# YooSungHyun/RNNTransducer

Hardware: AMD Instinct MI355X
Metric: utterances/sec (higher is better)
Workload: dtype f32

## Files before the change

### rnntransducer_amd/csrc/common.hpp

```cpp
#pragma once
#include <hip/hip_runtime.h>
#include <stdarg.h>
#include <stdint.h>
#include <stdio.h>

#include <atomic>

#include "rnnt_hip.h"

namespace rnnt {

void set_error(const char* fmt, ...);

#define RNNT_CHECK_ARG(cond, ...)      \
  do {                                 \
    if (!(cond)) {                     \
      ::rnnt::set_error(__VA_ARGS__);  \
      return RNNT_ERR_INVALID;         \
    }                                  \
  } while (0)

#define RNNT_CHECK_HIP(expr)                                                          \
  do {                                                                                \
    hipError_t e_ = (expr);                                                           \
// ... 2 lines not shown
      return RNNT_ERR_LAUNCH;                                                         \
    }                                                                                 \
  } while (0)

#define RNNT_CHECK_LAUNCH() RNNT_CHECK_HIP(hipGetLastError())

struct ProfScope {
  ProfScope(int kind, double work, hipStream_t s);
  ~ProfScope();
  int kind_;
  double work_;
  hipStream_t stream_;
  void* start_;
};

extern std::atomic<bool> g_launch_log_on;
void launch_log_note(const void* kernel, hipStream_t s);

static inline int64_t ceil_div(int64_t a, int64_t b) { return (a + b - 1) / b; }

int launch_colsum(const float* X, long M, long N, long ld, float* out, void* ws, size_t ws_bytes, hipStream_t s, int accumulate = 0);

size_t hp_plane_bytes(int64_t rows, int64_t K);
int hp_colmax(const float* x, int64_t rows, int64_t C, int64_t ld, uint32_t* amax, hipStream_t s);
int hp_split(const float* x, int64_t rows, int64_t K, int64_t ld, uint32_t* amax, void* planes, hipStream_t s, const int* rowidx = nullptr);
int hp_split_t(const float* x, int64_t R, int64_t K, int64_t ld, int64_t Ksrc, int64_t shift, const uint32_t* amax, void* planes,
               hipStream_t s, const int* kidx = nullptr);
int hp_split_both(const float* x, int64_t M, int64_t C, int64_t ld, const uint32_t* rowmax, const uint32_t* colmax, void* planes_rm,
                  void* planes_t, hipStream_t s, const int* rowidx = nullptr);
size_t hp_gemm_workspace_bytes(int64_t M, int64_t N, int64_t K);
int hp_gemm(const void* A, const uint32_t* a_amax, const void* B, const uint32_t* b_amax, int64_t M, int64_t N, int64_t K, float* C,
            int64_t c_div, int64_t c_so, int64_t c_si, const float* bias, unsigned flags, void* workspace, size_t workspace_bytes,
            hipStream_t s, const int* a_rowidx = nullptr, int64_t a_plane_rows = 0, const int* c_rowidx = nullptr);
struct HpProblem {
  const void* A; const uint32_t* a_amax; const void* B; const uint32_t* b_amax;
  int64_t M, N, K;
  float* C; int64_t ldc;
  unsigned flags;
};
constexpr int HP_GROUP_MAX = 4;
size_t hp_gemm_grouped_workspace_bytes(const int64_t* MN, int n);
int hp_gemm_grouped(const HpProblem* pr, int n, unsigned xcd_skip, unsigned* counter, void* workspace, size_t workspace_bytes,
                    hipStream_t s, unsigned* status = nullptr);
constexpr size_t HPQ_HEADER_BYTES = 256;
static inline size_t align_up(size_t a, size_t b) { return (a + b - 1) / b * b; }

__device__ __forceinline__ float gelu_tanh(float x) {
  const float k0 = 0.7978845608028654f, k1 = 0.044715f;
  float u = k0 * (x + k1 * x * x * x);
  return 0.5f * x * (1.0f + tanhf(u));
}
__device__ __forceinline__ float dgelu_tanh(float x) {
  const float k0 = 0.7978845608028654f, k1 = 0.044715f;
  float x2 = x * x;
  float u = k0 * (x + k1 * x * x2);
  float th = tanhf(u);
  float du = k0 * (1.0f + 3.0f * k1 * x2);
  return 0.5f * (1.0f + th) + 0.5f * x * (1.0f - th * th) * du;
}

__device__ __forceinline__ float sigmoidf_(float x) { return 1.0f / (1.0f + expf(-x)); }
__device__ __forceinline__ float tanh_e(float x) { return 1.0f - 2.0f / (expf(2.0f * x) + 1.0f); }
__device__ __forceinline__ float sigmoid_hw(float x) { return __builtin_amdgcn_rcpf(1.0f + __expf(-x)); }
__device__ __forceinline__ float tanh_hw(float x) { return 1.0f - 2.0f * __builtin_amdgcn_rcpf(__expf(2.0f * x) + 1.0f); }

typedef float f32x4 __attribute__((ext_vector_type(4)));
// ... 35 lines not shown
```

### rnntransducer_amd/csrc/gemm_hp.hip

```cpp
#include "common.hpp"

#include <stdlib.h>

namespace rnnt {
namespace {

typedef _Float16 f16x8 __attribute__((ext_vector_type(8)));
typedef __attribute__((address_space(3))) void lds_void;

constexpr int HP_BM = 256, HP_BN = 256, HP_BK = 32;
constexpr int HP_STAGE = (HP_BM + HP_BN) * 128;
constexpr int HP_RSRC = 0x00027000;

__device__ __forceinline__ float hp_scale_from_amax(unsigned amax_bits) {
  int eb = (int)((amax_bits >> 23) & 255u);
  if (eb == 0) return 1.0f;
  eb = eb < 15 ? 15 : eb;
  return __uint_as_float((unsigned)(268 - eb) << 23);
}
__device__ __forceinline__ float hp_inv_scale_from_amax(unsigned amax_bits) {
  int eb = (int)((amax_bits >> 23) & 255u);
  if (eb == 0) return 1.0f;
  eb = eb < 15 ? 15 : eb;
  return __uint_as_float((unsigned)(eb - 14) << 23);
// ... 391 lines not shown
      continue;
    }
#pragma unroll
    for (int ii = 0; ii < 4; ++ii) {
#pragma unroll
      for (int reg = 0; reg < 4; ++reg) {
        const int m = mrow + 16 * (4 * h + ii) + reg;
        const bool mok = m < p.M;
        const int mc = mok ? m : 0;
        float* crow = cbase + c_row(c_rowidx ? c_rowidx[mc] : mc);
        float old[4] = {0.f, 0.f, 0.f, 0.f};
        if (mode == 2) {
#pragma unroll
          for (int j = 0; j < 4; ++j)
            if (mok && nok[j]) old[j] = crow[ncol + 16 * j];
        }
#pragma unroll
        for (int j = 0; j < 4; ++j)
          if (mok && nok[j]) crow[ncol + 16 * j] = acc[4 * h + ii][j][reg] * sa[4 * ii + reg] * sb[j] + bias_v[j] + old[j];
      }
    }
  }
}

__device__ __forceinline__ int hp_grouped_tile(int idx, int tiles_m, int tiles_n, int group_m) {
  const int band = group_m * tiles_n;
  const int g = idx / band, r = idx - g * band;
  const int m_first = g * group_m;
  const int gm = min(tiles_m - m_first, group_m);
  const int n = r / gm, m = m_first + (r - n * gm);
  return n * tiles_m + m;
}

template <bool F16>
__global__ void __launch_bounds__(512, 1) gemm_hp_kernel(const HpGemmK p) {
  extern __shared__ __attribute__((aligned(16))) char lds[];
  int bid = hp_xcd_remap(blockIdx.x, p.tiles_m * p.tiles_n);
  if (p.group_m > 0) bid = hp_grouped_tile(bid, p.tiles_m, p.tiles_n, p.group_m);
  hp_tile256<F16, false>(p, bid, blockIdx.y, lds);
}

constexpr int HPQ_MAX = 4;
struct HpGemmQ {
  HpGemmK prob[HPQ_MAX];
  int unit_end[HPQ_MAX];
  int nprob;
  unsigned xcd_skip;
  unsigned* counter;
};

template <bool F16>
__global__ void __launch_bounds__(512, 1) gemm_hpq_kernel(const HpGemmQ q) {
  extern __shared__ __attribute__((aligned(16))) char lds[];
  unsigned xcc;
  asm volatile("s_getreg_b32 %0, hwreg(HW_REG_XCC_ID)" : "=s"(xcc));
  xcc &= 7u;
  if ((q.xcd_skip >> xcc) & 1u) return;
  const unsigned allow = ~q.xcd_skip & 0xffu;
  const int nq = __builtin_popcount(allow);
  const int mine = __builtin_popcount(allow & ((1u << xcc) - 1u));
  int* next = reinterpret_cast<int*>(lds + 2 * HP_STAGE);
  const int total = q.unit_end[q.nprob - 1];
  for (int hop = 0; hop < nq; ++hop) {
    const int qi = (mine + hop) % nq;
    const int lo = (int)((long)total * qi / nq), hi = (int)((long)total * (qi + 1) / nq);
    while (true) {
      if (threadIdx.x == 0) {
        const int got = lo + (int)atomicAdd(q.counter + qi, 1u);
        *next = got;
        if (got < hi) atomicAdd(q.counter + 8, 1u);
      }
      __syncthreads();
      const int u = __builtin_amdgcn_readfirstlane(*next);
      __syncthreads();
      if (u >= hi) break;
      int pi = 0;
      while (u >= q.unit_end[pi]) ++pi;
      const HpGemmK& p = q.prob[pi];
      const int local = u - (pi ? q.unit_end[pi - 1] : 0);
      const int tn = local % p.tiles_n, z = (local / p.tiles_n) % p.splits, tm = local / (p.tiles_n * p.splits);
      hp_tile256<F16, true>(p, tn * p.tiles_m + tm, z, lds);
    }
  }
}

__global__ void hpq_check_kernel(unsigned* counter, unsigned total, unsigned* status) {
  if (counter[8] != total) {
    counter[9] = 1u;
    if (status) __hip_atomic_store(status, 2u, __ATOMIC_RELAXED, __HIP_MEMORY_SCOPE_AGENT);
  }
}

__global__ void __launch_bounds__(256) hp_splitk_reduce_kernel(const HpGemmK p) {
  const long total = (long)p.M * p.N;
  for (long i = (long)blockIdx.x * 256 + threadIdx.x; i < total; i += (long)gridDim.x * 256) {
    const int m = (int)(i / p.N), n = (int)(i % p.N);
    float s = 0.f;
    for (int z = 0; z < p.splits; ++z) s += p.slab[(long)z * total + i];
    if (p.bias) s += p.bias[n];
    const int mo = p.c_rowidx ? p.c_rowidx[m] : m;
    const long off = (long)(mo / p.c_div) * p.c_so + (long)(mo % p.c_div) * p.c_si + n;
    if (p.flags & RNNT_GEMM_ACCUM) s += p.C[off];
    p.C[off] = s;
  }
}

}

size_t hp_plane_bytes(int64_t rows, int64_t K) { return (size_t)rows * (size_t)ceil_div(K, 32) * 128; }

int hp_colmax(const float* x, int64_t rows, int64_t C, int64_t ld, uint32_t* amax, hipStream_t s) {
  RNNT_CHECK_HIP(hipMemsetAsync(amax, 0, (size_t)C * 4, s));
  if (rows == 0 || C == 0) return RNNT_OK;
  long chunks = ceil_div(2048, ceil_div(C, 256));
  if (chunks > ceil_div(rows, 64)) chunks = ceil_div(rows, 64);
  if (chunks < 1) chunks = 1;
  const long rpc = ceil_div(rows, chunks);
  ProfScope prof(RNNT_K_HP_SPLIT, 4.0 * (double)rows * (double)C, s);
  hipLaunchKernelGGL(hp_colmax_kernel, dim3((unsigned)ceil_div(C, 256), (unsigned)ceil_div(rows, rpc)), dim3(256), 0, s, x, (long)rows, (int)C,
                     (long)ld, rpc, amax);
  RNNT_CHECK_LAUNCH();
  return RNNT_OK;
}

int hp_split(const float* x, int64_t rows, int64_t K, int64_t ld, uint32_t* amax, void* planes, hipStream_t s, const int* rowidx) {
  if (rows == 0) return RNNT_OK;
  const long blocks = ceil_div(rows, 4);
  ProfScope prof(RNNT_K_HP_SPLIT, 8.0 * (double)rows * (double)K, s);
  hipLaunchKernelGGL(hp_split_kernel, dim3((unsigned)(blocks < 8192 ? blocks : 8192)), dim3(256), 0, s, x, (long)rows, (int)K, (long)ld, amax,
                     (char*)planes, rowidx);
  RNNT_CHECK_LAUNCH();
  return RNNT_OK;
}

int hp_split_t(const float* x, int64_t R, int64_t K, int64_t ld, int64_t Ksrc, int64_t shift, const uint32_t* amax, void* planes,
               hipStream_t s, const int* kidx) {
  if (R == 0 || K == 0) return RNNT_OK;
  ProfScope prof(RNNT_K_HP_SPLIT, 8.0 * (double)R * (double)K, s);
  hipLaunchKernelGGL(hp_split_t_kernel, dim3((unsigned)ceil_div(K, 32), (unsigned)ceil_div(R, 256)), dim3(256), 0, s, x, (int)R, (int)K, (long)ld,
                     (int)Ksrc, (int)shift, amax, (char*)planes, kidx);
  RNNT_CHECK_LAUNCH();
  return RNNT_OK;
}

int hp_split_both(const float* x, int64_t M, int64_t C, int64_t ld, const uint32_t* rowmax, const uint32_t* colmax, void* planes_rm,
                  void* planes_t, hipStream_t s, const int* rowidx) {
  if (M == 0 || C == 0) return RNNT_OK;
  ProfScope prof(RNNT_K_HP_SPLIT, 12.0 * (double)M * (double)C, s);
  hipLaunchKernelGGL(hp_split_both_kernel, dim3((unsigned)ceil_div(M, 32), (unsigned)ceil_div(C, 256)), dim3(256), 0, s, x, (int)M, (int)C, (long)ld,
                     rowmax, colmax, (char*)planes_rm, (char*)planes_t, rowidx);
  RNNT_CHECK_LAUNCH();
  return RNNT_OK;
}

struct HpGemmPlan {
  int tiles_m, tiles_n, group_m, splits, kt_per_split;
  size_t workspace_bytes_wanted;
};
static HpGemmPlan hp_gemm_plan(int64_t M, int64_t N, int64_t K, size_t workspace_bytes) {
  HpGemmPlan pl;
  pl.tiles_m = (int)ceil_div(M, HP_BM); pl.tiles_n = (int)ceil_div(N, HP_BN);
  const long tiles = (long)pl.tiles_m * pl.tiles_n;
  const long nkt = ceil_div(K, HP_BK);
  {
    static const int env_gm = getenv("RNNT_GEMM_HP_GROUP_M") ? atoi(getenv("RNNT_GEMM_HP_GROUP_M")) : -1;
    pl.group_m = env_gm >= 0 ? env_gm : (tiles >= 256 ? 8 : 4);
  }
  long want = 1;
  if (tiles < 192 && nkt >= 64) {
    want = ceil_div(256, tiles);
    if (want > nkt / 32) want = nkt / 32;
    if (want > 32) want = 32;
    if (want < 2) want = 1;
  }
  const size_t slab = (size_t)M * (size_t)N * 4;
  pl.workspace_bytes_wanted = want >= 2 ? (size_t)want * slab : 0;
  const size_t by_ws = workspace_bytes / slab;
  long splits = (size_t)want > by_ws ? (long)by_ws : want;
  if (splits < 2) splits = 1;
  pl.kt_per_split = (int)ceil_div(nkt, splits);
  pl.splits = (int)ceil_div(nkt, pl.kt_per_split);
  return pl;
}

size_t hp_gemm_workspace_bytes(int64_t M, int64_t N, int64_t K) { return hp_gemm_plan(M, N, K, 0).workspace_bytes_wanted; }

int hp_gemm(const void* A, const uint32_t* a_amax, const void* B, const uint32_t* b_amax, int64_t M, int64_t N, int64_t K, float* C,
            int64_t c_div, int64_t c_so, int64_t c_si, const float* bias, unsigned flags, void* workspace, size_t workspace_bytes,
            hipStream_t s, const int* a_rowidx, int64_t a_plane_rows, const int* c_rowidx) {
  RNNT_CHECK_ARG(A && B && C && a_amax && b_amax, "gemm_hp: null operand");
  RNNT_CHECK_ARG(!a_rowidx || a_plane_rows >= M, "gemm_hp: a gathered A operand needs the row count of its planes");
  RNNT_CHECK_ARG(M >= 1 && N >= 1 && K >= 1 && M < (1ll << 31) && N < (1ll << 31) && K < (1ll << 31), "gemm_hp: bad dims");
  RNNT_CHECK_ARG(c_div >= 1, "gemm_hp: c_div must be >= 1");
  RNNT_CHECK_ARG(((reinterpret_cast<uintptr_t>(A) | reinterpret_cast<uintptr_t>(B)) & 127) == 0, "gemm_hp: planes must be 128-byte aligned");
  HpGemmK k;
  k.M = (int)M; k.N = (int)N; k.nkt = (int)ceil_div(K, HP_BK);
  const size_t ab = hp_plane_bytes(a_rowidx ? a_plane_rows : M, K), bb = hp_plane_bytes(N, K);
  RNNT_CHECK_ARG(ab < (1ull << 32) && bb < (1ull << 32), "gemm_hp: an operand exceeds the 4 GB a buffer resource addresses");
  k.A = (const char*)A; k.a_pitch = (unsigned)k.nkt * 128u; k.a_bytes = (unsigned)ab;
  k.B = (const char*)B; k.b_pitch = (unsigned)k.nkt * 128u; k.b_bytes = (unsigned)bb;
  k.a_amax = a_amax; k.b_amax = b_amax;
  k.C = C; k.c_div = (int)(c_div > 0x7fffffff ? 0x7fffffff : c_div); k.c_so = c_so; k.c_si = c_si;
  k.bias = bias; k.flags = flags;
  k.a_rowidx = a_rowidx; k.c_rowidx = c_rowidx;
  const bool f16 = (flags & RNNT_GEMM_HP_F16) != 0u;
  const HpGemmPlan pl = hp_gemm_plan(M, N, K, workspace ? workspace_bytes : 0);
  k.tiles_m = pl.tiles_m; k.tiles_n = pl.tiles_n; k.group_m = pl.group_m;
  k.splits = pl.splits; k.kt_per_split = pl.kt_per_split;
  const int tiles = k.tiles_m * k.tiles_n, splits = k.splits;
  k.slab = (float*)workspace;
  if (f16) RNNT_CHECK_HIP(hipFuncSetAttribute((const void*)gemm_hp_kernel<true>, hipFuncAttributeMaxDynamicSharedMemorySize, 2 * HP_STAGE));
  else RNNT_CHECK_HIP(hipFuncSetAttribute((const void*)gemm_hp_kernel<false>, hipFuncAttributeMaxDynamicSharedMemorySize, 2 * HP_STAGE));
  {
    ProfScope prof(RNNT_K_GEMM_HP, 2.0 * (double)M * (double)N * (double)K, s);
    if (f16) hipLaunchKernelGGL(gemm_hp_kernel<true>, dim3(tiles, splits), dim3(512), 2 * HP_STAGE, s, k);
    else hipLaunchKernelGGL(gemm_hp_kernel<false>, dim3(tiles, splits), dim3(512), 2 * HP_STAGE, s, k);
    RNNT_CHECK_LAUNCH();
    if (splits > 1) {
      const long blocks = ceil_div((long)M * N, 256);
      hipLaunchKernelGGL(hp_splitk_reduce_kernel, dim3((unsigned)(blocks < 2048 ? blocks : 2048)), dim3(256), 0, s, k);
      RNNT_CHECK_LAUNCH();
    }
  }
  return RNNT_OK;
}

constexpr int HPQ_SPLIT_CAP = 8;
size_t hp_gemm_grouped_workspace_bytes(const int64_t* MN, int n) {
  size_t total = 0;
  for (int i = 0; i < n; ++i) total += align_up((size_t)HPQ_SPLIT_CAP * (size_t)MN[i] * 4, 256);
  return total;
}

int hp_gemm_grouped(const HpProblem* pr, int n, unsigned xcd_skip, unsigned* counter, void* workspace, size_t workspace_bytes,
                    hipStream_t s, unsigned* status) {
  RNNT_CHECK_ARG(pr && n >= 1 && n <= HPQ_MAX && counter, "gemm_hp grouped: 1..%d problems and a counter word", HPQ_MAX);
  RNNT_CHECK_ARG((xcd_skip & 0xffu) != 0xffu, "gemm_hp grouped: xcd_skip leaves no XCD");
  const bool f16 = (pr[0].flags & RNNT_GEMM_HP_F16) != 0u;
  for (int i = 1; i < n; ++i)
    RNNT_CHECK_ARG(((pr[i].flags & RNNT_GEMM_HP_F16) != 0u) == f16, "gemm_hp grouped: the problems of one launch share RNNT_GEMM_HP_F16");
  HpGemmQ q = {};
  q.nprob = n; q.xcd_skip = xcd_skip; q.counter = counter;
  int xcds = 0;
  for (int x = 0; x < 8; ++x) xcds += !((xcd_skip >> x) & 1u);
  const long workers = 32l * xcds;
  long total_kt = 0;
  double flops = 0.0;
  for (int i = 0; i < n; ++i) {
    const HpProblem& a = pr[i];
    RNNT_CHECK_ARG(a.A && a.B && a.C && a.a_amax && a.b_amax, "gemm_hp grouped: null operand (problem %d)", i);
    RNNT_CHECK_ARG(a.M >= 1 && a.N >= 1 && a.K >= 1 && a.M < (1ll << 31) && a.N < (1ll << 31) && a.K < (1ll << 31) && a.ldc >= a.N,
                   "gemm_hp grouped: bad dims (problem %d)", i);
    RNNT_CHECK_ARG(((reinterpret_cast<uintptr_t>(a.A) | reinterpret_cast<uintptr_t>(a.B)) & 127) == 0, "gemm_hp grouped: planes must be 128-byte aligned");
    HpGemmK& k = q.prob[i];
    k.M = (int)a.M; k.N = (int)a.N; k.nkt = (int)ceil_div(a.K, HP_BK);
    const size_t ab = hp_plane_bytes(a.M, a.K), bb = hp_plane_bytes(a.N, a.K);
    RNNT_CHECK_ARG(ab < (1ull << 32) && bb < (1ull << 32), "gemm_hp grouped: an operand exceeds the 4 GB a buffer resource addresses");
// ... 11 lines not shown
  if (chunk < 32) chunk = 32;
  size_t off = 0;
  int units = 0;
  for (int i = 0; i < n; ++i) {
    HpGemmK& k = q.prob[i];
    long splits = ceil_div(k.nkt, chunk);
    if (splits > HPQ_SPLIT_CAP) splits = HPQ_SPLIT_CAP;
    const size_t per = (size_t)k.M * k.N * 4;
    while (splits > 1 && (!workspace || off + align_up((size_t)splits * per, 256) > workspace_bytes)) --splits;
    k.kt_per_split = (int)ceil_div(k.nkt, splits);
    k.splits = (int)ceil_div(k.nkt, k.kt_per_split);
    k.slab = k.splits > 1 ? reinterpret_cast<float*>((char*)workspace + off) : nullptr;
    if (k.splits > 1) off += align_up((size_t)k.splits * per, 256);
    units += k.tiles_m * k.tiles_n * k.splits;
    q.unit_end[i] = units;
  }
  RNNT_CHECK_HIP(hipMemsetAsync(counter, 0, 64, s));
  const int lds = 2 * HP_STAGE + 16;
  const void* qk = f16 ? (const void*)gemm_hpq_kernel<true> : (const void*)gemm_hpq_kernel<false>;
  RNNT_CHECK_HIP(hipFuncSetAttribute(qk, hipFuncAttributeMaxDynamicSharedMemorySize, lds));
  {
    ProfScope prof(RNNT_K_GEMM_HP, flops, s);
    int cus = 0, dev = 0;
    if (hipGetDevice(&dev) != hipSuccess || hipDeviceGetAttribute(&cus, hipDeviceAttributeMultiprocessorCount, dev) != hipSuccess || cus < 8) cus = 256;
    const dim3 grid(!xcd_skip && units < cus ? units : cus);
    if (f16) hipLaunchKernelGGL(gemm_hpq_kernel<true>, grid, dim3(512), lds, s, q);
    else hipLaunchKernelGGL(gemm_hpq_kernel<false>, grid, dim3(512), lds, s, q);
    RNNT_CHECK_LAUNCH();
    hipLaunchKernelGGL(hpq_check_kernel, dim3(1), dim3(1), 0, s, counter, (unsigned)units, status);
    RNNT_CHECK_LAUNCH();
    for (int i = 0; i < n; ++i)
      if (q.prob[i].splits > 1) {
        const long blocks = ceil_div((long)q.prob[i].M * q.prob[i].N, 256);
        hipLaunchKernelGGL(hp_splitk_reduce_kernel, dim3((unsigned)(blocks < 2048 ? blocks : 2048)), dim3(256), 0, s, q.prob[i]);
        RNNT_CHECK_LAUNCH();
      }
  }
  return RNNT_OK;
}

}

using namespace rnnt;

extern "C" size_t rnnt_hip_hp_bytes(int64_t rows, int64_t K) {
  if (rows < 0 || K < 0) return 0;
  return hp_plane_bytes(rows, K);
}

extern "C" int rnnt_hip_hp_split_ex(const float* x, int64_t rows, int64_t K, int64_t ld, int32_t transpose, int64_t src_rows, int64_t shift,
                                    void* planes, uint32_t* amax, int32_t amax_given, const int32_t* idx, void* stream) {
  RNNT_CHECK_ARG(x && planes && amax && rows >= 0 && K >= 0, "hp_split: bad arguments");
  RNNT_CHECK_ARG(rows < (1ll << 31) && K < (1ll << 31), "hp_split: dims must fit 31 bits");
  RNNT_CHECK_ARG((reinterpret_cast<uintptr_t>(planes) & 127) == 0, "hp_split: planes must be 128-byte aligned");
  hipStream_t s = (hipStream_t)stream;
  if (!transpose) {
    RNNT_CHECK_ARG(ld >= K, "hp_split: ld < K");
    RNNT_CHECK_ARG(!amax_given, "hp_split: the row-major split computes its row maxima itself");
    return hp_split(x, rows, K, ld, amax, planes, s, idx);
  }
  RNNT_CHECK_ARG(ld >= rows && src_rows >= 1, "hp_split: transposed source is (src_rows x >= rows), ld >= rows");
  RNNT_CHECK_ARG(src_rows < (1ll << 31) && shift > -(1ll << 31) && shift < (1ll << 31), "hp_split: src_rows and shift must fit 31 bits");
  if (!amax_given)
    if (int rc = hp_colmax(x, src_rows, rows, ld, amax, s)) return rc;
  return hp_split_t(x, rows, K, ld, src_rows, shift, amax, planes, s, idx);
}

// ... 78 lines not shown
```

### rnntransducer_amd/csrc/lstm_layer.hip

```cpp
#include "lstm_shared.hpp"

#include <string.h>

namespace rnnt {
namespace {

__global__ void db_reduce_kernel(const float* __restrict__ part, int rows_per_dir, int H, int ngate, float* __restrict__ o0,
                                 float* __restrict__ o1, int accumulate, float* __restrict__ p0 = nullptr,
                                 float* __restrict__ p1 = nullptr) {
  const int c = blockIdx.x * 256 + threadIdx.x, d = blockIdx.y;
  if (c >= 4 * H || (c & 3) >= ngate) return;
  const float* src = part + (long)d * rows_per_dir * 4 * H + c;
  float s = 0.f;
  for (int r = 0; r < rows_per_dir; ++r) s += src[(long)r * 4 * H];
  float* o = (d ? o1 : o0) + (c & 3) * H + (c >> 2);
  *o = accumulate ? *o + s : s;
  float* q = d ? p1 : p0;
  if (q) {
    q += (c & 3) * H + (c >> 2);
    *q = accumulate ? *q + s : s;
  }
}
__global__ void permute_w_kernel(const float* __restrict__ w0, const float* __restrict__ w1, int H, int I, int ngate,
                                 float* __restrict__ out) {
// ... 143 lines not shown
  uint32_t* amax_xt;
  uint32_t* amax_yt;
  uint32_t* amax_dgh_cols;
  size_t total;
};

LstmWs carve_lstm(void* ws, int T, int B, int I, int H, int D, const LayerPlan& lp) {
  LstmWs w;
  char* p = reinterpret_cast<char*>(ws);
  size_t off = 0;
  auto take = [&](size_t bytes) { char* q = p ? p + off : nullptr; off += align_up(bytes, 256); return q; };
  w.nflags = lp.nflags;
  w.sync_bytes = align_up((2 * w.nflags + 16) * 4, 16);
  w.flags = reinterpret_cast<unsigned*>(take(w.sync_bytes));
  w.hx_bytes = lp.hx_bytes;
  w.hx = reinterpret_cast<float*>(take(w.hx_bytes));
  w.wp = reinterpret_cast<float*>(take((size_t)D * 4 * H * I * 4));
  w.bp = reinterpret_cast<float*>(take((size_t)D * 4 * H * 4));
  w.dwhh = reinterpret_cast<float*>(take((size_t)D * 4 * H * H * 4));
  w.dbg = reinterpret_cast<unsigned long long*>(take(512 * 8 * 8));
  w.dbp_half = (size_t)D * (B + 64) * 4 * H;
  w.dbp = reinterpret_cast<float*>(take(2 * w.dbp_half * 4));
  const int64_t M = (int64_t)T * B, N4 = (int64_t)D * 4 * H;
  size_t sc = rnnt_hip_gemm_workspace_bytes(N4, I, M);
  const size_t s2 = rnnt_hip_gemm_workspace_bytes(4 * H, H, M > B ? M - B : 1);
  const size_t s3 = rnnt_hip_colsum_workspace_bytes(M, N4);
  if (s2 > sc) sc = s2;
  if (s3 > sc) sc = s3;
  w.hp = lp.hp;
  if (w.hp) {
    const size_t h1 = hp_gemm_workspace_bytes(N4, I, M), h2 = hp_gemm_workspace_bytes(4 * H, H, M);
    if (h1 > sc) sc = h1;
    if (h2 > sc) sc = h2;
    const int64_t mn[3] = {N4 * I, (int64_t)4 * H * H, (int64_t)4 * H * H};
    const size_t h3 = HPQ_HEADER_BYTES + hp_gemm_grouped_workspace_bytes(mn, 1 + D);
    if (h3 > sc) sc = h3;
  }
  w.scratch_bytes = sc;
  w.scratch = take(sc);
  w.hp_x = w.hp_w = w.hp_dg = w.hp_dgt = w.hp_yt = nullptr;
  w.amax_x = w.amax_w = w.amax_dg_rows = w.amax_dg_cols = w.amax_wt = w.amax_xt = w.amax_yt = w.amax_dgh_cols = nullptr;
  if (w.hp) {
    uint32_t* hp_amax = reinterpret_cast<uint32_t*>(take((size_t)(2 * M + 3 * N4 + 2 * I + (int64_t)D * H) * 4));
    if (hp_amax) {
      w.amax_x = hp_amax;
      w.amax_w = hp_amax + M;
      w.amax_dg_rows = hp_amax + M + N4;
      w.amax_dg_cols = hp_amax + 2 * M + N4;
      w.amax_wt = hp_amax + 2 * M + 2 * N4;
      w.amax_xt = hp_amax + 2 * M + 2 * N4 + I;
      w.amax_yt = hp_amax + 2 * M + 2 * N4 + 2 * I;
      w.amax_dgh_cols = hp_amax + 2 * M + 2 * N4 + 2 * I + (int64_t)D * H;
    }
    w.hp_x = take(hp_plane_bytes(M, I) > hp_plane_bytes(I, M) ? hp_plane_bytes(M, I) : hp_plane_bytes(I, M));
    w.hp_w = take(hp_plane_bytes(N4, I) > hp_plane_bytes(I, N4) ? hp_plane_bytes(N4, I) : hp_plane_bytes(I, N4));
    w.hp_dg = take(hp_plane_bytes(M, N4));
    w.hp_dgt = take(hp_plane_bytes(N4, M));
    w.hp_yt = take((size_t)D * hp_plane_bytes(H, M));
  }
  w.total = off;
  return w;
}

int check_desc(const rnnt_lstm_desc* d, LayerPlan* lp, LstmWs* w) {
  RNNT_CHECK_ARG(d != nullptr, "lstm: null descriptor");
  RNNT_CHECK_ARG(d->T >= 1 && d->I >= 1, "lstm: T and I must be positive (T=%d I=%d)", d->T, d->I);
// ... 190 lines not shown
  RNNT_CHECK_ARG(bd->dy, "lstm_bwd: null dy");
  const int T = d->T, B = d->B, H = d->H, D = d->D, I = d->I;
  const bool gru = d->cell == RNNT_CELL_GRU;
  const int ngate = gate_count(d->cell);
  RNNT_CHECK_ARG(!gru || d->aux, "lstm_bwd: GRU needs the aux buffer (T,B,D*4H)");
  for (int k = 0; k < D; ++k) RNNT_CHECK_ARG(!gru || bd->db_hh[k], "lstm_bwd: GRU needs db_hh");
  const int acc = bd->accumulate ? 1 : 0;
  float* twin0 = gru ? nullptr : bd->db_hh[0];
  float* twin1 = gru ? nullptr : second(bd->db_hh, D);
  if (twin0 == bd->db[0]) twin0 = nullptr;
  if (twin1 == second(bd->db, D)) twin1 = nullptr;
  const float* ghid = gru ? d->aux : d->gates;
  RNNT_CHECK_ARG(x_is_plain(d), "lstm_bwd: x must be time-major contiguous (T,B,I)");
  for (int k = 0; k < D; ++k) RNNT_CHECK_ARG(bd->dw_ih[k] && bd->dw_hh[k] && bd->db[k], "lstm_bwd: null gradient output");
  hipStream_t s = (hipStream_t)stream;
  RNNT_CHECK_ARG(bd->phase >= RNNT_LSTM_BWD_ALL && bd->phase <= RNNT_LSTM_BWD_WEIGHTS, "lstm_bwd: phase must be 0, 1 or 2");
  const bool do_recur = bd->phase != RNNT_LSTM_BWD_WEIGHTS, do_weights = bd->phase != RNNT_LSTM_BWD_RECUR;

  const bool f16 = precision == RNNT_PRECISION_F16 && lp.takes_f16;
  const unsigned hpf = f16 ? RNNT_GEMM_HP_F16 : 0u;
  const bool ragged = ragged_call(d, lp);
  const int* ridx = ragged ? d->row_idx : nullptr;
  const int64_t M = (int64_t)T * B, N4 = (int64_t)D * 4 * H;
  const int64_t Mv = ragged ? d->n_rows : M;
  const bool hp_in = w.hp && I >= 128;
  const bool hp_dwih = hp_in || (w.hp && I >= 32 && !getenv("RNNT_GEMM_HP_NO_NARROW"));
  const bool fused_db = lp.form == Form::V34 || lp.form == Form::V5;
  const int db_rows = lp.p2.G * 4 * lp.p2.BQ;
  const bool v5_maxima = lp.form == Form::V5 && w.hp;
  const bool both = v5_maxima && !gru && hp_in && bd->dx && !getenv("RNNT_GEMM_HP_NO_FUSED_SPLIT");
  const unsigned xcd_skip =
      (lp.form == Form::V5 && bd->beside_recurrence && lp.recurrence_xcds <= 4 && lp.cus == 256) ? (1u << lp.recurrence_xcds) - 1u : 0u;
  const bool grouped = hp_in && T > 1 && !gru && (xcd_skip != 0u || getenv("RNNT_GEMM_HP_GROUP")) && !getenv("RNNT_GEMM_HP_NO_GROUP");
  int rc = RNNT_OK;

  if (do_recur)
    if ((rc = reset_exchange(w, s))) return rc;
  LstmK k;
  fill_kernel_args(d, lp, w, &k);
  k.dy = bd->dy;
  k.gbound = ragged ? 1 : 0;
  if (v5_maxima) {
    k.colmax = w.amax_dg_cols;
    k.colmax_h = w.amax_dgh_cols;
    if (both) k.rowmax = w.amax_dg_rows;
    unsigned* first = both ? k.rowmax : k.colmax;
    if (do_recur) RNNT_CHECK_HIP(hipMemsetAsync(first, 0, (size_t)(w.amax_dgh_cols + N4 - first) * 4, s));
  }
  if (do_recur || lp.form == Form::NONE)
    if ((rc = launch_recurrence(lp, k, true, f16, s))) return rc;

  if (w.hp) {
    if (do_recur && hp_in && bd->dx) {
      if (both) rc = hp_split_both(d->gates, Mv, N4, N4, w.amax_dg_rows, w.amax_dg_cols, w.hp_dg, w.hp_dgt, s, ridx);
      else rc = hp_split(d->gates, Mv, N4, N4, w.amax_dg_rows, w.hp_dg, s, ridx);
      if (rc) return rc;
    }
    if (do_weights && !v5_maxima)
      if ((rc = hp_colmax(d->gates, M, N4, N4, w.amax_dg_cols, s))) return rc;
    if (do_weights && !both)
      if ((rc = hp_split_t(d->gates, N4, Mv, N4, M, 0, w.amax_dg_cols, w.hp_dgt, s, ridx))) return rc;
  }
  if (do_recur && bd->dx) {
    if ((rc = permute_w_ih(d, w, s))) return rc;
    if (hp_in) {
      if ((rc = hp_colmax(w.wp, N4, I, I, w.amax_wt, s))) return rc;
      if ((rc = hp_split_t(w.wp, I, N4, I, N4, 0, w.amax_wt, w.hp_w, s))) return rc;
      if ((rc = hp_gemm(w.hp_dg, w.amax_dg_rows, w.hp_w, w.amax_wt, Mv, I, N4, bd->dx, 1, I, 0, nullptr, hpf, nullptr, 0, s, ridx, M, ridx))) return rc;
    } else {
      rnnt_gemm_desc g = {};
      g.M = M; g.N = I; g.K = N4;
      g.A = d->gates; g.a_div = 1; g.a_so = N4; g.a_si = 0; g.a_sk = 1; g.a_mc = 0;
      g.B = w.wp; g.b_sn = 1; g.b_sk = I;
      g.C = bd->dx; g.c_div = 1; g.c_so = I; g.c_si = 0;
      if ((rc = rnnt_hip_gemm_f32(&g, s))) return rc;
    }
    if (ragged) {
      hipLaunchKernelGGL(zero_padded_rows_kernel, dim3((unsigned)(ceil_div(M, 4) < 2048 ? ceil_div(M, 4) : 2048)), dim3(256), 0, s, bd->dx, d->lens, T, B, I);
      RNNT_CHECK_LAUNCH();
    }
  }
  if (!do_weights) return RNNT_OK;
  if (hp_dwih) {
    if (d->x_abs_bound > 0.f) {
      uint32_t bits;
      memcpy(&bits, &d->x_abs_bound, 4);
      RNNT_CHECK_HIP(hipMemsetD32Async((hipDeviceptr_t)w.amax_xt, (int)bits, (size_t)I, s));
    } else if ((rc = hp_colmax(d->x, M, I, I, w.amax_xt, s))) return rc;
    if ((rc = hp_split_t(d->x, I, Mv, I, M, 0, w.amax_xt, w.hp_x, s, ridx))) return rc;
    if (!grouped)
      if ((rc = hp_gemm(w.hp_dgt, w.amax_dg_cols, w.hp_x, w.amax_xt, N4, I, Mv, w.wp, 1, I, 0, nullptr, hpf, w.scratch, w.scratch_bytes, s))) return rc;
  } else {
    rnnt_gemm_desc g = {};
    g.M = N4; g.N = I; g.K = M;
    g.A = d->gates; g.a_mc = 1; g.a_sk = N4; g.a_div = 1;
    g.B = d->x; g.b_sn = 1; g.b_sk = I;
    g.C = w.wp; g.c_div = 1; g.c_so = I; g.c_si = 0;
    g.workspace = w.scratch; g.workspace_bytes = w.scratch_bytes;
    if ((rc = rnnt_hip_gemm_f32(&g, s))) return rc;
  }
  if (!grouped)
    if ((rc = unpermute(w.wp, H, I, D, ngate, bd->dw_ih, acc, s))) return rc;
  if (w.hp && T > 1) {
    if (d->cell != RNNT_CELL_RNN_RELU) {
      RNNT_CHECK_HIP(hipMemsetD32Async((hipDeviceptr_t)w.amax_yt, 0x3f800000, (size_t)D * H, s));
    } else if ((rc = hp_colmax(d->y, M, (int64_t)D * H, (int64_t)D * H, w.amax_yt, s))) return rc;
    uint32_t* a_dgh = w.amax_dg_cols;
    if (gru) {
      if (v5_maxima) a_dgh = w.amax_dgh_cols;
      else if ((rc = hp_colmax(ghid, M, N4, N4, a_dgh, s))) return rc;
      if ((rc = hp_split_t(ghid, N4, Mv, N4, M, 0, a_dgh, w.hp_dgt, s, ridx))) return rc;
    }
    HpProblem pr[HP_GROUP_MAX];
    int npr = 0;
    if (grouped) pr[npr++] = HpProblem{w.hp_dgt, w.amax_dg_cols, w.hp_x, w.amax_xt, N4, I, Mv, w.wp, I, hpf};
    for (int dir = 0; dir < D; ++dir) {
      char* yt = w.hp_yt + (size_t)dir * hp_plane_bytes(H, M);
      uint32_t* a_y = w.amax_yt + (int64_t)dir * H;
      float* dwhh = w.dwhh + (int64_t)dir * 4 * H * H;
      if ((rc = hp_split_t(d->y + (int64_t)dir * H, H, Mv, (int64_t)D * H, M, dir == 0 ? -B : B, a_y, yt, s, ridx))) return rc;
      const char* ag = w.hp_dgt + (size_t)dir * 4 * H * (size_t)ceil_div(Mv, 32) * 128;
      if (grouped) {
        pr[npr++] = HpProblem{ag, a_dgh + (int64_t)dir * 4 * H, yt, a_y, 4 * H, H, Mv, dwhh, H, hpf};
        continue;
      }
      if ((rc = hp_gemm(ag, a_dgh + (int64_t)dir * 4 * H, yt, a_y, 4 * H, H, Mv, dwhh, 1, H, 0, nullptr, hpf, w.scratch, w.scratch_bytes, s)))
        return rc;
    }
    if (grouped) {
      if ((rc = hp_gemm_grouped(pr, npr, xcd_skip, reinterpret_cast<unsigned*>(w.scratch), (char*)w.scratch + HPQ_HEADER_BYTES,
                                w.scratch_bytes - HPQ_HEADER_BYTES, s, k.status)))
        return rc;
      if ((rc = unpermute(w.wp, H, I, D, ngate, bd->dw_ih, acc, s))) return rc;
    }
  } else
  for (int dir = 0; dir < D; ++dir) {
    rnnt_gemm_desc g = {};
    g.M = 4 * H; g.N = H; g.K = (int64_t)(T - 1) * B;
    const int64_t shift_g = dir == 0 ? (int64_t)B * N4 : 0;
    const int64_t shift_y = dir == 0 ? 0 : (int64_t)B * D * H;
    g.A = ghid + shift_g + (int64_t)dir * 4 * H; g.a_mc = 1; g.a_sk = N4; g.a_div = 1;
    g.B = d->y + shift_y + (int64_t)dir * H; g.b_sn = 1; g.b_sk = (int64_t)D * H;
    g.C = w.dwhh + (int64_t)dir * 4 * H * H; g.c_div = 1; g.c_so = H; g.c_si = 0;
    g.workspace = w.scratch; g.workspace_bytes = w.scratch_bytes;
    if (g.K > 0) {
      if ((rc = rnnt_hip_gemm_f32(&g, s))) return rc;
    } else {
      RNNT_CHECK_HIP(hipMemsetAsync(g.C, 0, (size_t)4 * H * H * 4, s));
    }
  }
  if ((rc = unpermute(w.dwhh, H, H, D, ngate, bd->dw_hh, acc, s))) return rc;
  if (fused_db) {
    hipLaunchKernelGGL(db_reduce_kernel, dim3((unsigned)ceil_div(4 * H, 256), D), dim3(256), 0, s, k.dbp, db_rows, H, ngate, bd->db[0],
                       second(bd->db, D), acc, twin0, twin1);
    RNNT_CHECK_LAUNCH();
    if (gru) {
      hipLaunchKernelGGL(db_reduce_kernel, dim3((unsigned)ceil_div(4 * H, 256), D), dim3(256), 0, s, k.dbhp, db_rows, H, ngate, bd->db_hh[0],
                         second(bd->db_hh, D), acc);
      RNNT_CHECK_LAUNCH();
    }
  } else {
    if ((rc = launch_colsum(d->gates, (long)M, (long)N4, (long)N4, w.bp, w.scratch, w.scratch_bytes, s))) return rc;
    if ((rc = unpermute(w.bp, H, 1, D, ngate, bd->db, acc, s, twin0, twin1))) return rc;
    if (gru) {
      if ((rc = launch_colsum(ghid, (long)M, (long)N4, (long)N4, w.bp, w.scratch, w.scratch_bytes, s))) return rc;
      if ((rc = unpermute(w.bp, H, 1, D, ngate, bd->db_hh, acc, s))) return rc;
    }
  }
  return RNNT_OK;
}

extern "C" int rnnt_hip_lstm_bwd(const rnnt_lstm_bwd_desc* bd, void* stream) { return lstm_bwd_impl(bd, RNNT_PRECISION_FP32, stream); }

extern "C" int rnnt_hip_lstm_bwd_ex(const rnnt_lstm_bwd_desc* bd, uint32_t precision, void* stream) {
  RNNT_CHECK_ARG(precision == RNNT_PRECISION_FP32 || precision == RNNT_PRECISION_F16, "lstm_bwd_ex: precision must be 0 (fp32) or 1 (f16), got %u",
                 precision);
  return lstm_bwd_impl(bd, precision, stream);
}

extern "C" int rnnt_hip_lstm_check(const void* workspace, void* stream) {
  RNNT_CHECK_ARG(workspace != nullptr, "lstm_check: null workspace");
  unsigned st = 0;
  RNNT_CHECK_HIP(hipMemcpyAsync(&st, workspace, sizeof(st), hipMemcpyDeviceToHost, (hipStream_t)stream));
  RNNT_CHECK_HIP(hipStreamSynchronize((hipStream_t)stream));
// ... 18 lines not shown
```

Measured before the change: 1341.

## Batch per-direction LSTM weight-gradient GEMMs and write directly in PyTorch layout

Adds a batched variant of the split-bf16 GEMM that runs up to two same-shape problems in one launch via blockIdx.z, with split-K planning and reduction aware of the batch. For LSTM backward, the dW_ih and dW_hh GEMMs for both directions are issued as single batched launches. Their output goes straight into the final gradient buffers using the C-row divisor/stride mapping, with ACCUM applied there. This removes the separate unpermute passes and halves GEMM launch count. The batched launch also exposes more tiles, which lowers split-K factors. Risks: the c_div=4 mapping must reproduce the old unpermute gate ordering, and the hp_dwih condition guarding skipped unpermute may not match every path.

Result: no change. 1349, median of 6 (+0.6%).

```diff
diff --git a/rnntransducer_amd/csrc/common.hpp b/rnntransducer_amd/csrc/common.hpp
--- a/rnntransducer_amd/csrc/common.hpp
+++ b/rnntransducer_amd/csrc/common.hpp
@@ -58,6 +58,15 @@
 int hp_gemm(const void* A, const uint32_t* a_amax, const void* B, const uint32_t* b_amax, int64_t M, int64_t N, int64_t K, float* C,
             int64_t c_div, int64_t c_so, int64_t c_si, const float* bias, unsigned flags, void* workspace, size_t workspace_bytes,
             hipStream_t s, const int* a_rowidx = nullptr, int64_t a_plane_rows = 0, const int* c_rowidx = nullptr);
+struct HpOperands {
+  const void* A; const uint32_t* a_amax; const void* B; const uint32_t* b_amax;
+  float* C;
+};
+constexpr int HP_BATCH_MAX = 2;
+size_t hp_gemm_batched_workspace_bytes(int64_t M, int64_t N, int64_t K, int nprob);
+int hp_gemm_batched(const HpOperands* op, int nprob, int64_t M, int64_t N, int64_t K, int64_t c_div, int64_t c_so, int64_t c_si,
+                    const float* bias, unsigned flags, void* workspace, size_t workspace_bytes, hipStream_t s,
+                    const int* a_rowidx = nullptr, int64_t a_plane_rows = 0, const int* c_rowidx = nullptr);
 struct HpProblem {
   const void* A; const uint32_t* a_amax; const void* B; const uint32_t* b_amax;
   int64_t M, N, K;
diff --git a/rnntransducer_amd/csrc/gemm_hp.hip b/rnntransducer_amd/csrc/gemm_hp.hip
--- a/rnntransducer_amd/csrc/gemm_hp.hip
+++ b/rnntransducer_amd/csrc/gemm_hp.hip
@@ -447,9 +447,26 @@
   return n * tiles_m + m;
 }
 
+struct HpGemmB {
+  HpGemmK p;
+  const char* A1; const char* B1;
+  const unsigned* a_amax1; const unsigned* b_amax1;
+  float* C1;
+  int nprob;
+};
+__device__ __forceinline__ HpGemmK hp_batch_problem(const HpGemmB& b, int pb) {
+  HpGemmK p = b.p;
+  if (pb) {
+    p.A = b.A1; p.B = b.B1; p.a_amax = b.a_amax1; p.b_amax = b.b_amax1; p.C = b.C1;
+    if (p.splits > 1) p.slab += (long)p.splits * p.M * p.N;
+  }
+  return p;
+}
+
 template <bool F16>
-__global__ void __launch_bounds__(512, 1) gemm_hp_kernel(const HpGemmK p) {
+__global__ void __launch_bounds__(512, 1) gemm_hp_kernel(const HpGemmB b) {
   extern __shared__ __attribute__((aligned(16))) char lds[];
+  const HpGemmK p = hp_batch_problem(b, blockIdx.z);
   int bid = hp_xcd_remap(blockIdx.x, p.tiles_m * p.tiles_n);
   if (p.group_m > 0) bid = hp_grouped_tile(bid, p.tiles_m, p.tiles_n, p.group_m);
   hp_tile256<F16, false>(p, bid, blockIdx.y, lds);
@@ -506,17 +523,22 @@
   }
 }
 
-__global__ void __launch_bounds__(256) hp_splitk_reduce_kernel(const HpGemmK p) {
-  const long total = (long)p.M * p.N;
+__global__ void __launch_bounds__(256) hp_splitk_reduce_kernel(const HpGemmB b) {
+  const HpGemmK& p = b.p;
+  const long per = (long)p.M * p.N, total = per * b.nprob;
   for (long i = (long)blockIdx.x * 256 + threadIdx.x; i < total; i += (long)gridDim.x * 256) {
-    const int m = (int)(i / p.N), n = (int)(i % p.N);
+    const int pb = i >= per ? 1 : 0;
+    const long e = i - (pb ? per : 0l);
+    const int m = (int)(e / p.N), n = (int)(e % p.N);
+    const float* slab = p.slab + (pb ? (long)p.splits * per : 0l);
+    float* Cb = pb ? b.C1 : p.C;
     float s = 0.f;
-    for (int z = 0; z < p.splits; ++z) s += p.slab[(long)z * total + i];
+    for (int z = 0; z < p.splits; ++z) s += slab[(long)z * per + e];
     if (p.bias) s += p.bias[n];
     const int mo = p.c_rowidx ? p.c_rowidx[m] : m;
     const long off = (long)(mo / p.c_div) * p.c_so + (long)(mo % p.c_div) * p.c_si + n;
-    if (p.flags & RNNT_GEMM_ACCUM) s += p.C[off];
-    p.C[off] = s;
+    if (p.flags & RNNT_GEMM_ACCUM) s += Cb[off];
+    Cb[off] = s;
   }
 }
 
@@ -572,23 +594,24 @@
   int tiles_m, tiles_n, group_m, splits, kt_per_split;
   size_t workspace_bytes_wanted;
 };
-static HpGemmPlan hp_gemm_plan(int64_t M, int64_t N, int64_t K, size_t workspace_bytes) {
+static HpGemmPlan hp_gemm_plan(int64_t M, int64_t N, int64_t K, size_t workspace_bytes, int nprob = 1) {
   HpGemmPlan pl;
   pl.tiles_m = (int)ceil_div(M, HP_BM); pl.tiles_n = (int)ceil_div(N, HP_BN);
   const long tiles = (long)pl.tiles_m * pl.tiles_n;
+  const long launch_tiles = tiles * nprob;
   const long nkt = ceil_div(K, HP_BK);
   {
     static const int env_gm = getenv("RNNT_GEMM_HP_GROUP_M") ? atoi(getenv("RNNT_GEMM_HP_GROUP_M")) : -1;
     pl.group_m = env_gm >= 0 ? env_gm : (tiles >= 256 ? 8 : 4);
   }
   long want = 1;
-  if (tiles < 192 && nkt >= 64) {
-    want = ceil_div(256, tiles);
+  if (launch_tiles < 192 && nkt >= 64) {
+    want = ceil_div(256, launch_tiles);
     if (want > nkt / 32) want = nkt / 32;
     if (want > 32) want = 32;
     if (want < 2) want = 1;
   }
-  const size_t slab = (size_t)M * (size_t)N * 4;
+  const size_t slab = (size_t)nprob * (size_t)M * (size_t)N * 4;
   pl.workspace_bytes_wanted = want >= 2 ? (size_t)want * slab : 0;
   const size_t by_ws = workspace_bytes / slab;
   long splits = (size_t)want > by_ws ? (long)by_ws : want;
@@ -599,27 +622,38 @@
 }
 
 size_t hp_gemm_workspace_bytes(int64_t M, int64_t N, int64_t K) { return hp_gemm_plan(M, N, K, 0).workspace_bytes_wanted; }
-
-int hp_gemm(const void* A, const uint32_t* a_amax, const void* B, const uint32_t* b_amax, int64_t M, int64_t N, int64_t K, float* C,
-            int64_t c_div, int64_t c_so, int64_t c_si, const float* bias, unsigned flags, void* workspace, size_t workspace_bytes,
-            hipStream_t s, const int* a_rowidx, int64_t a_plane_rows, const int* c_rowidx) {
-  RNNT_CHECK_ARG(A && B && C && a_amax && b_amax, "gemm_hp: null operand");
+size_t hp_gemm_batched_workspace_bytes(int64_t M, int64_t N, int64_t K, int nprob) {
+  return hp_gemm_plan(M, N, K, 0, nprob).workspace_bytes_wanted;
+}
+
+int hp_gemm_batched(const HpOperands* op, int nprob, int64_t M, int64_t N, int64_t K, int64_t c_div, int64_t c_so, int64_t c_si,
+                    const float* bias, unsigned flags, void* workspace, size_t workspace_bytes, hipStream_t s, const int* a_rowidx,
+                    int64_t a_plane_rows, const int* c_rowidx) {
+  RNNT_CHECK_ARG(op && nprob >= 1 && nprob <= HP_BATCH_MAX, "gemm_hp: 1..%d problems per launch", HP_BATCH_MAX);
+  for (int i = 0; i < nprob; ++i) RNNT_CHECK_ARG(op[i].A && op[i].B && op[i].C && op[i].a_amax && op[i].b_amax, "gemm_hp: null operand");
   RNNT_CHECK_ARG(!a_rowidx || a_plane_rows >= M, "gemm_hp: a gathered A operand needs the row count of its planes");
   RNNT_CHECK_ARG(M >= 1 && N >= 1 && K >= 1 && M < (1ll << 31) && N < (1ll << 31) && K < (1ll << 31), "gemm_hp: bad dims");
   RNNT_CHECK_ARG(c_div >= 1, "gemm_hp: c_div must be >= 1");
-  RNNT_CHECK_ARG(((reinterpret_cast<uintptr_t>(A) | reinterpret_cast<uintptr_t>(B)) & 127) == 0, "gemm_hp: planes must be 128-byte aligned");
-  HpGemmK k;
+  for (int i = 0; i < nprob; ++i)
+    RNNT_CHECK_ARG(((reinterpret_cast<uintptr_t>(op[i].A) | reinterpret_cast<uintptr_t>(op[i].B)) & 127) == 0,
+                   "gemm_hp: planes must be 128-byte aligned");
+  HpGemmB b = {};
+  HpGemmK& k = b.p;
   k.M = (int)M; k.N = (int)N; k.nkt = (int)ceil_div(K, HP_BK);
   const size_t ab = hp_plane_bytes(a_rowidx ? a_plane_rows : M, K), bb = hp_plane_bytes(N, K);
   RNNT_CHECK_ARG(ab < (1ull << 32) && bb < (1ull << 32), "gemm_hp: an operand exceeds the 4 GB a buffer resource addresses");
-  k.A = (const char*)A; k.a_pitch = (unsigned)k.nkt * 128u; k.a_bytes = (unsigned)ab;
-  k.B = (const char*)B; k.b_pitch = (unsigned)k.nkt * 128u; k.b_bytes = (unsigned)bb;
-  k.a_amax = a_amax; k.b_amax = b_amax;
-  k.C = C; k.c_div = (int)(c_div > 0x7fffffff ? 0x7fffffff : c_div); k.c_so = c_so; k.c_si = c_si;
+  k.A = (const char*)op[0].A; k.a_pitch = (unsigned)k.nkt * 128u; k.a_bytes = (unsigned)ab;
+  k.B = (const char*)op[0].B; k.b_pitch = (unsigned)k.nkt * 128u; k.b_bytes = (unsigned)bb;
+  k.a_amax = op[0].a_amax; k.b_amax = op[0].b_amax;
+  k.C = op[0].C; k.c_div = (int)(c_div > 0x7fffffff ? 0x7fffffff : c_div); k.c_so = c_so; k.c_si = c_si;
   k.bias = bias; k.flags = flags;
   k.a_rowidx = a_rowidx; k.c_rowidx = c_rowidx;
+  b.nprob = nprob;
+  if (nprob > 1) {
+    b.A1 = (const char*)op[1].A; b.B1 = (const char*)op[1].B; b.a_amax1 = op[1].a_amax; b.b_amax1 = op[1].b_amax; b.C1 = op[1].C;
+  }
   const bool f16 = (flags & RNNT_GEMM_HP_F16) != 0u;
-  const HpGemmPlan pl = hp_gemm_plan(M, N, K, workspace ? workspace_bytes : 0);
+  const HpGemmPlan pl = hp_gemm_plan(M, N, K, workspace ? workspace_bytes : 0, nprob);
   k.tiles_m = pl.tiles_m; k.tiles_n = pl.tiles_n; k.group_m = pl.group_m;
   k.splits = pl.splits; k.kt_per_split = pl.kt_per_split;
   const int tiles = k.tiles_m * k.tiles_n, splits = k.splits;
@@ -627,17 +661,24 @@
   if (f16) RNNT_CHECK_HIP(hipFuncSetAttribute((const void*)gemm_hp_kernel<true>, hipFuncAttributeMaxDynamicSharedMemorySize, 2 * HP_STAGE));
   else RNNT_CHECK_HIP(hipFuncSetAttribute((const void*)gemm_hp_kernel<false>, hipFuncAttributeMaxDynamicSharedMemorySize, 2 * HP_STAGE));
   {
-    ProfScope prof(RNNT_K_GEMM_HP, 2.0 * (double)M * (double)N * (double)K, s);
-    if (f16) hipLaunchKernelGGL(gemm_hp_kernel<true>, dim3(tiles, splits), dim3(512), 2 * HP_STAGE, s, k);
-    else hipLaunchKernelGGL(gemm_hp_kernel<false>, dim3(tiles, splits), dim3(512), 2 * HP_STAGE, s, k);
+    ProfScope prof(RNNT_K_GEMM_HP, 2.0 * (double)nprob * (double)M * (double)N * (double)K, s);
+    if (f16) hipLaunchKernelGGL(gemm_hp_kernel<true>, dim3(tiles, splits, nprob), dim3(512), 2 * HP_STAGE, s, b);
+    else hipLaunchKernelGGL(gemm_hp_kernel<false>, dim3(tiles, splits, nprob), dim3(512), 2 * HP_STAGE, s, b);
     RNNT_CHECK_LAUNCH();
     if (splits > 1) {
-      const long blocks = ceil_div((long)M * N, 256);
-      hipLaunchKernelGGL(hp_splitk_reduce_kernel, dim3((unsigned)(blocks < 2048 ? blocks : 2048)), dim3(256), 0, s, k);
+      const long blocks = ceil_div((long)nprob * M * N, 256);
+      hipLaunchKernelGGL(hp_splitk_reduce_kernel, dim3((unsigned)(blocks < 2048 ? blocks : 2048)), dim3(256), 0, s, b);
       RNNT_CHECK_LAUNCH();
     }
   }
   return RNNT_OK;
+}
+
+int hp_gemm(const void* A, const uint32_t* a_amax, const void* B, const uint32_t* b_amax, int64_t M, int64_t N, int64_t K, float* C,
+            int64_t c_div, int64_t c_so, int64_t c_si, const float* bias, unsigned flags, void* workspace, size_t workspace_bytes,
+            hipStream_t s, const int* a_rowidx, int64_t a_plane_rows, const int* c_rowidx) {
+  const HpOperands op = {A, a_amax, B, b_amax, C};
+  return hp_gemm_batched(&op, 1, M, N, K, c_div, c_so, c_si, bias, flags, workspace, workspace_bytes, s, a_rowidx, a_plane_rows, c_rowidx);
 }
 
 constexpr int HPQ_SPLIT_CAP = 8;
@@ -715,7 +756,9 @@
     for (int i = 0; i < n; ++i)
       if (q.prob[i].splits > 1) {
         const long blocks = ceil_div((long)q.prob[i].M * q.prob[i].N, 256);
-        hipLaunchKernelGGL(hp_splitk_reduce_kernel, dim3((unsigned)(blocks < 2048 ? blocks : 2048)), dim3(256), 0, s, q.prob[i]);
+        HpGemmB one = {};
+        one.p = q.prob[i]; one.nprob = 1;
+        hipLaunchKernelGGL(hp_splitk_reduce_kernel, dim3((unsigned)(blocks < 2048 ? blocks : 2048)), dim3(256), 0, s, one);
         RNNT_CHECK_LAUNCH();
       }
   }
diff --git a/rnntransducer_amd/csrc/lstm_layer.hip b/rnntransducer_amd/csrc/lstm_layer.hip
--- a/rnntransducer_amd/csrc/lstm_layer.hip
+++ b/rnntransducer_amd/csrc/lstm_layer.hip
@@ -199,6 +199,9 @@
     const size_t h1 = hp_gemm_workspace_bytes(N4, I, M), h2 = hp_gemm_workspace_bytes(4 * H, H, M);
     if (h1 > sc) sc = h1;
     if (h2 > sc) sc = h2;
+    const size_t h4 = hp_gemm_batched_workspace_bytes(4 * H, I, M, D), h5 = hp_gemm_batched_workspace_bytes(4 * H, H, M, D);
+    if (h4 > sc) sc = h4;
+    if (h5 > sc) sc = h5;
     const int64_t mn[3] = {N4 * I, (int64_t)4 * H * H, (int64_t)4 * H * H};
     const size_t h3 = HPQ_HEADER_BYTES + hp_gemm_grouped_workspace_bytes(mn, 1 + D);
     if (h3 > sc) sc = h3;
@@ -455,6 +458,8 @@
   const unsigned xcd_skip =
       (lp.form == Form::V5 && bd->beside_recurrence && lp.recurrence_xcds <= 4 && lp.cus == 256) ? (1u << lp.recurrence_xcds) - 1u : 0u;
   const bool grouped = hp_in && T > 1 && !gru && (xcd_skip != 0u || getenv("RNNT_GEMM_HP_GROUP")) && !getenv("RNNT_GEMM_HP_NO_GROUP");
+  const bool fused_dw = w.hp && d->cell == RNNT_CELL_LSTM && !grouped && !getenv("RNNT_LSTM_DW_UNFUSED");
+  const unsigned dwf = hpf | (acc ? RNNT_GEMM_ACCUM : 0u);
   int rc = RNNT_OK;
 
   if (do_recur)
@@ -511,7 +516,13 @@
       RNNT_CHECK_HIP(hipMemsetD32Async((hipDeviceptr_t)w.amax_xt, (int)bits, (size_t)I, s));
     } else if ((rc = hp_colmax(d->x, M, I, I, w.amax_xt, s))) return rc;
     if ((rc = hp_split_t(d->x, I, Mv, I, M, 0, w.amax_xt, w.hp_x, s, ridx))) return rc;
-    if (!grouped)
+    if (fused_dw) {
+      HpOperands op[HP_BATCH_MAX];
+      for (int dir = 0; dir < D; ++dir)
+        op[dir] = HpOperands{w.hp_dgt + (size_t)dir * 4 * H * (size_t)ceil_div(Mv, 32) * 128, w.amax_dg_cols + (int64_t)dir * 4 * H, w.hp_x,
+                             w.amax_xt, bd->dw_ih[dir]};
+      if ((rc = hp_gemm_batched(op, D, 4 * H, I, Mv, 4, I, (int64_t)H * I, nullptr, dwf, w.scratch, w.scratch_bytes, s))) return rc;
+    } else if (!grouped)
       if ((rc = hp_gemm(w.hp_dgt, w.amax_dg_cols, w.hp_x, w.amax_xt, N4, I, Mv, w.wp, 1, I, 0, nullptr, hpf, w.scratch, w.scratch_bytes, s))) return rc;
   } else {
     rnnt_gemm_desc g = {};
@@ -522,7 +533,7 @@
     g.workspace = w.scratch; g.workspace_bytes = w.scratch_bytes;
     if ((rc = rnnt_hip_gemm_f32(&g, s))) return rc;
   }
-  if (!grouped)
+  if (!grouped && !(fused_dw && hp_dwih))
     if ((rc = unpermute(w.wp, H, I, D, ngate, bd->dw_ih, acc, s))) return rc;
   if (w.hp && T > 1) {
     if (d->cell != RNNT_CELL_RNN_RELU) {
@@ -535,6 +546,7 @@
       if ((rc = hp_split_t(ghid, N4, Mv, N4, M, 0, a_dgh, w.hp_dgt, s, ridx))) return rc;
     }
     HpProblem pr[HP_GROUP_MAX];
+    HpOperands op[HP_BATCH_MAX];
     int npr = 0;
     if (grouped) pr[npr++] = HpProblem{w.hp_dgt, w.amax_dg_cols, w.hp_x, w.amax_xt, N4, I, Mv, w.wp, I, hpf};
     for (int dir = 0; dir < D; ++dir) {
@@ -547,9 +559,15 @@
         pr[npr++] = HpProblem{ag, a_dgh + (int64_t)dir * 4 * H, yt, a_y, 4 * H, H, Mv, dwhh, H, hpf};
         continue;
       }
+      if (fused_dw) {
+        op[dir] = HpOperands{ag, a_dgh + (int64_t)dir * 4 * H, yt, a_y, bd->dw_hh[dir]};
+        continue;
+      }
       if ((rc = hp_gemm(ag, a_dgh + (int64_t)dir * 4 * H, yt, a_y, 4 * H, H, Mv, dwhh, 1, H, 0, nullptr, hpf, w.scratch, w.scratch_bytes, s)))
         return rc;
     }
+    if (fused_dw)
+      if ((rc = hp_gemm_batched(op, D, 4 * H, H, Mv, 4, H, (int64_t)H * H, nullptr, dwf, w.scratch, w.scratch_bytes, s))) return rc;
     if (grouped) {
       if ((rc = hp_gemm_grouped(pr, npr, xcd_skip, reinterpret_cast<unsigned*>(w.scratch), (char*)w.scratch + HPQ_HEADER_BYTES,
                                 w.scratch_bytes - HPQ_HEADER_BYTES, s, k.status)))
@@ -572,7 +590,8 @@
       RNNT_CHECK_HIP(hipMemsetAsync(g.C, 0, (size_t)4 * H * H * 4, s));
     }
   }
-  if ((rc = unpermute(w.dwhh, H, H, D, ngate, bd->dw_hh, acc, s))) return rc;
+  if (!(fused_dw && T > 1))
+    if ((rc = unpermute(w.dwhh, H, H, D, ngate, bd->dw_hh, acc, s))) return rc;
   if (fused_db) {
     hipLaunchKernelGGL(db_reduce_kernel, dim3((unsigned)ceil_div(4 * H, 256), D), dim3(256), 0, s, k.dbp, db_rows, H, ngate, bd->db[0],
                        second(bd->db, D), acc, twin0, twin1);
```
